# yanglei18/SGV3D

Measured on AMD Instinct MI355X. Metric: camera frames/sec at 864x1536->BEV, higher is better.
Workload: dtype f32

## Files before the change

### include/sgv3d_hip.h

```cpp
#ifndef SGV3D_HIP_H
#define SGV3D_HIP_H

#include <stddef.h>
#include <stdint.h>

#ifdef __cplusplus
extern "C" {
#endif

#define SGV3D_OK 0
#define SGV3D_EINVAL (-1)
#define SGV3D_ELAUNCH (-2)
#define SGV3D_ENOSPACE (-3)

const char *sgv3d_last_error(void);
int sgv3d_abi_version(void);


int sgv3d_voxel_pooling_forward(int batch_size, int num_points, int num_channels,
                                int num_voxel_x, int num_voxel_y, int num_voxel_z,
                                const int32_t *geom_xyz, const float *input_features,
                                float *output_features, int32_t *pos_memo, void *stream);
int sgv3d_voxel_pooling_forward_fresh(int batch_size, int num_points, int num_channels,
                                      int num_voxel_x, int num_voxel_y, int num_voxel_z,
// ... 112 lines not shown

#define SGV3D_TILE_128x128 1
#define SGV3D_TILE_128x64 2
#define SGV3D_TILE_64x128 3
#define SGV3D_TILE_64x64 4
#define SGV3D_TILE_32x128 9
#define SGV3D_TILE_48x64 10
#define SGV3D_TILE_X3 64
#define SGV3D_TILE_MFIRST 16
#define SGV3D_TILE_OCC5 32
#define SGV3D_WINOGRAD_RESIDENT 6
#define SGV3D_WINOGRAD_HALF 8

int sgv3d_conv_winograd4_pack_weight(const float *w_src , int cout, int cin, int k_pad, int cout_pad,
                                     float *u_packed , void *stream);
int sgv3d_conv_winograd4_pack_weight_x3(const float *w_src, int cout, int cin, int cin_pad, int cout_pad, void *u3_packed,
                                        void *stream);

int sgv3d_conv_pack_weight_x3(const float *w_src, int cout, int cin, int kh, int kw, int cin_pad, int cout_pad, void *u3_packed,
                              void *stream);
int sgv3d_conv2d_x3_forward(const sgv3d_conv_desc *desc, const float *x, const void *u3_packed, const float *scale,
                            const float *bias, const float *residual, float *y, void *workspace, size_t workspace_bytes,
                            void *stream);
int sgv3d_conv2d_x3_shortcut_forward(const sgv3d_conv_desc *desc_a, const float *xa, const void *u3a, const float *scale_a,
                                     const float *bias_a, const sgv3d_conv_desc *desc_b, const float *xb, const void *u3b,
                                     const float *scale_b, const float *bias_b, float *y, void *stream);
int sgv3d_stem_pool_x3_forward(int batch, int h, int w, const float *x_nchw, const void *w_x3, size_t w_bytes, const float *scale,
                               const float *shift, float *y_nhwc, int y_ld, int variant, void *stream);
int sgv3d_wino4_lattice_axis(int n, int dil, int tile, int k0, int count, int *tiles, int *stacked, int *pixels);
size_t sgv3d_conv2d_winograd4_workspace_bytes(const sgv3d_conv_desc *desc );
int sgv3d_conv2d_winograd4_forward(const sgv3d_conv_desc *desc , const float *x, const float *u_packed,
                                   const float *scale, const float *bias, const float *residual, float *y,
                                   void *workspace, size_t workspace_bytes, void *stream);

size_t sgv3d_conv2d_winograd4_multi_workspace_bytes(int n, const sgv3d_conv_desc *descs );
int sgv3d_conv2d_winograd4_forward_multi(int n, const sgv3d_conv_desc *descs , const float *x, const void *const *u_packed,
                                         const float *const *scale, const float *const *bias, float *const *y, void *workspace,
                                         size_t workspace_bytes, void *stream);

void sgv3d_conv_pack_geometry(int k, int n, int *k_pad, int *n_pad);

int sgv3d_conv_pack_weight(const float *w_src, int cout, int cin, int kh, int kw, int cin_pad,
                           int transposed, int k_order, float *w_packed, int k_pad, int cout_pad,
                           void *stream);

size_t sgv3d_conv2d_workspace_bytes(const sgv3d_conv_desc *desc );
// ... 660 lines not shown
```

### sgv3d_amd/_lib.py

```python
import ctypes
import os

_HERE = os.path.dirname(os.path.abspath(__file__))
LIB_PATH = os.path.join(_HERE, "csrc", "libsgv3d_hip.so")

c_int, c_void_p, c_size_t, c_ll = ctypes.c_int, ctypes.c_void_p, ctypes.c_size_t, ctypes.c_longlong


class ConvDesc(ctypes.Structure):
    _fields_ = [(n, c_int) for n in (
        "batch", "in_h", "in_w", "cin", "out_h", "out_w", "cout", "kh", "kw", "stride", "pad", "dil",
        "x_ld", "x_coff", "y_ld", "y_coff", "res_ld", "relu", "mode", "deconv_ks", "k_pad", "cout_pad",
        "tile", "x_nchw", "k_order", "split_k")]


class VitAttnDesc(ctypes.Structure):
    _fields_ = [(n, c_int) for n in ("batch", "height", "width", "heads", "head_dim", "win_h", "win_w")]


class SamAttnDesc(ctypes.Structure):
    _fields_ = [(n, c_int) for n in ("batch", "nq", "nk", "heads", "head_dim", "q_ld", "k_ld", "v_ld", "o_ld")] + [("scale", ctypes.c_float)]


CONV_NORMAL, CONV_DECONV, CONV_NCHW_OUT, CONV_GROUP_PLANES = 0, 1, 2, 3
# ... 59 lines not shown
    "sgv3d_scale_channels_bf16": (c_int, [c_int] * 3 + [c_void_p] * 4),
    "sgv3d_global_avgpool_bf16": (c_int, [c_int] * 4 + [c_void_p] * 3 + [c_size_t, c_void_p]),
    "sgv3d_broadcast_channels_bf16": (c_int, [c_int] * 5 + [c_void_p] * 3),
    "sgv3d_upsample_bilinear2x_bf16": (c_int, [c_int] * 4 + [c_void_p] * 3),
    "sgv3d_add_mul_sigmoid_bf16": (c_int, [c_ll] + [c_void_p] * 5),
    "sgv3d_deform_im2col3x3_bf16": (c_int, [c_int] * 5 + [c_void_p] * 2 + [c_int, c_void_p, c_void_p]),
    "sgv3d_conv3x3_patch_bf16_weight_bytes": (c_size_t, [c_int, c_int]),
    "sgv3d_conv3x3_patch_bf16_debug_stamps": (None, [c_void_p]),
    "sgv3d_conv3x3_patch_bf16_pack_weight": (c_int, [c_void_p, c_int, c_int, c_void_p, c_void_p]),
    "sgv3d_conv3x3_patch_bf16_forward": (c_int, [c_int] * 11 + [c_void_p] * 6 + [c_int, c_int, c_void_p, c_size_t, c_void_p]),
    "sgv3d_conv_dw_bf16_weight_bytes": (c_size_t, [c_int] * 4),
    "sgv3d_conv_dw_bf16_pack_weight": (c_int, [c_void_p] + [c_int] * 5 + [c_void_p, c_void_p]),
    "sgv3d_conv_dw_bf16_forward": (c_int, [ctypes.POINTER(ConvDesc)] + [c_void_p] * 7),
    "sgv3d_conv_dw_bf16_workspace_bytes": (c_size_t, [ctypes.POINTER(ConvDesc)]),
    "sgv3d_conv_dw_bf16_forward_splitk": (c_int, [ctypes.POINTER(ConvDesc)] + [c_void_p] * 7 + [c_size_t, c_void_p]),
    "sgv3d_conv_dw_bf16_pair_forward": (c_int, [ctypes.POINTER(ConvDesc)] + [c_void_p] * 4 + [c_int] + [c_void_p] * 4 + [c_int, c_void_p, c_int, c_int, c_int, c_void_p]),
    "sgv3d_conv_winograd_weight_floats": (c_size_t, [c_int, c_int]),
    "sgv3d_conv_winograd_pack_weight": (c_int, [c_void_p, c_int, c_int, c_int, c_void_p, c_void_p]),
    "sgv3d_conv2d_winograd_forward": (c_int, [ctypes.POINTER(ConvDesc)] + [c_void_p] * 8 + [c_size_t, c_void_p]),
    "sgv3d_conv_winograd4_pack_weight": (c_int, [c_void_p, c_int, c_int, c_int, c_int, c_void_p, c_void_p]),
    "sgv3d_conv_winograd4_pack_weight_x3": (c_int, [c_void_p, c_int, c_int, c_int, c_int, c_void_p, c_void_p]),
    "sgv3d_conv_pack_weight_x3": (c_int, [c_void_p, c_int, c_int, c_int, c_int, c_int, c_int, c_void_p, c_void_p]),
    "sgv3d_conv2d_x3_forward": (c_int, [c_void_p] * 8 + [c_size_t, c_void_p]),
    "sgv3d_conv2d_x3_shortcut_forward": (c_int, [c_void_p] * 12),
    "sgv3d_stem_pool_x3_forward": (c_int, [c_int] * 3 + [c_void_p, c_void_p, c_size_t] + [c_void_p] * 3 + [c_int, c_int, c_void_p]),
    "sgv3d_wino4_lattice_axis": (c_int, [c_int] * 5 + [c_void_p] * 3),
    "sgv3d_conv2d_winograd4_workspace_bytes": (c_size_t, [ctypes.POINTER(ConvDesc)]),
    "sgv3d_conv2d_winograd4_forward": (c_int, [ctypes.POINTER(ConvDesc)] + [c_void_p] * 7 + [c_size_t, c_void_p]),
    "sgv3d_conv2d_winograd4_multi_workspace_bytes": (c_size_t, [c_int, c_void_p]),
    "sgv3d_conv2d_winograd4_forward_multi": (c_int, [c_int] + [c_void_p] * 7 + [c_size_t, c_void_p]),
    "sgv3d_maxpool3x3s2": (c_int, [c_int] * 4 + [c_void_p] * 3),
    "sgv3d_maxpool3x3s2_bf16": (c_int, [c_int] * 4 + [c_void_p] * 3),
    "sgv3d_nchw_to_nhwc": (c_int, [c_int] * 5 + [c_void_p] * 3),
    "sgv3d_nhwc_to_nchw": (c_int, [c_int] * 6 + [c_void_p] * 3),
    "sgv3d_global_avgpool_workspace_bytes": (c_size_t, [c_int] * 2),
    "sgv3d_global_avgpool": (c_int, [c_int] * 4 + [c_void_p] * 3 + [c_size_t, c_void_p]),
    "sgv3d_dense": (c_int, [c_int] * 3 + [c_void_p] * 4 + [c_int, c_void_p, c_void_p]),
    "sgv3d_broadcast_channels": (c_int, [c_int] * 5 + [c_void_p] * 3),
    "sgv3d_scale_channels": (c_int, [c_int] * 3 + [c_void_p] * 4),
    "sgv3d_copy_channels": (c_int, [c_int] * 5 + [c_void_p] * 3),
    "sgv3d_upsample_bilinear2x": (c_int, [c_int] * 4 + [c_void_p] * 3),
    "sgv3d_add_mul_sigmoid": (c_int, [c_ll] + [c_void_p] * 5),
    "sgv3d_bsm_compose": (c_int, [c_int] * 6 + [c_void_p, c_int, ctypes.c_float, c_void_p, c_void_p]),
    "sgv3d_deform_im2col3x3": (c_int, [c_int] * 5 + [c_void_p, c_void_p, c_int, c_void_p, c_void_p]),
    "sgv3d_deform_conv3x3_forward": (c_int, [c_int] * 6 + [c_void_p, c_void_p, c_int, c_void_p, c_int, c_int, c_void_p, c_int, c_int,
                                                          c_void_p]),
# ... 226 lines not shown
```

### sgv3d_amd/csrc/conv_pw_x3.hip

```cpp
#include "conv_common.hpp"
#include "f32x3.hpp"

using namespace sgv3d;

namespace {

struct PwX3Args {
    const float *x, *scale, *bias, *res;
    const void *w;
    float *y;
    int M, K, N;
    int x_ld, x_coff, y_ld, y_coff, res_ld, relu;
    int cout_pad, tiles_m, tiles_n, mfirst;
    unsigned x_bytes, w_bytes;
    int in_h, in_w, out_h, out_w, kh, kw, stride, pad, dil;
    int cin4;
    int split_k;
    float *ws;
    const float *x2, *scale2, *bias2;
    const void *w2;
    int K2, x2_ld, x2_coff;
    unsigned x2_bytes, w2_bytes;
};

template <int MA, int WN, int MODE>
__global__ __launch_bounds__(64 * WN, 2) void conv_pw_x3_kernel(const PwX3Args a) {
    constexpr bool TAPS = MODE == 1, TM = MODE == 2, DUAL = MODE == 3, DECONV = MODE == 4;
    constexpr int NT = 64 * WN, BM = 16 * MA, BN = 32 * WN;
    constexpr int PLANE = x3_plane_bytes(BM), BUF = x3_buf_bytes(BM);
    __shared__ __attribute__((aligned(16))) unsigned char smem[2 * BUF];

    const int logical = xcd_tile(blockIdx.x, a.tiles_m * a.tiles_n);
    int tn, tm;
    if (a.mfirst) {
        tm = (int)((unsigned)logical / (unsigned)a.tiles_n);
        tn = logical - tm * a.tiles_n;
    } else {
        tn = (int)((unsigned)logical / (unsigned)a.tiles_m);
        tm = logical - tn * a.tiles_m;
    }
    const int m0 = tm * BM, n0 = tn * BN;
    const int kb = a.K >> 5;

    const int tid = threadIdx.x;
    __amdgpu_buffer_rsrc_t x_rsrc = __builtin_amdgcn_make_buffer_rsrc(const_cast<float *>(a.x), 0, (int)a.x_bytes, 0x00020000);
    __amdgpu_buffer_rsrc_t w_rsrc = __builtin_amdgcn_make_buffer_rsrc(const_cast<void *>(a.w), 0, (int)a.w_bytes, 0x00020000);
// ... 150 lines not shown
#pragma unroll
        for (int i = 0; i < PA; ++i) {
            const int r = arow + RPA * i;
            const bool live = a_on[i] && m0 + r < a.M;
            const int m = live ? m0 + r : 0;
            const int t = (int)((unsigned)m / (unsigned)a.out_w);
            const int ow = m - t * a.out_w;
            const int n = (int)((unsigned)t / (unsigned)a.out_h);
            const int oh = t - n * a.out_h;
            xg[i] = live ? (unsigned)((((long long)(n * a.in_h + oh * a.stride) * a.in_w + ow * a.stride) * a.x2_ld + a.x2_coff + ach * 4) * 4)
                         : 0xffffffffu;
        }
#pragma unroll
        for (int nb = 0; nb < 2; ++nb) wgo[nb] = u3_lane_offset((n0 >> 4) + 2 * wave + nb, nkt, lane, a.cout_pad);
        __syncthreads();
        PWX3_KLOOP();
    }
#undef PWX3_KLOOP
#undef PWX3_REQUEST
#undef PWX3_STORE

    if (a.split_k > 1) {
        float *wsb = a.ws + (size_t)blockIdx.y * a.M * a.N;
#pragma unroll
        for (int nb = 0; nb < 2; ++nb) {
            const int col = n0 + 32 * wave + 16 * nb + 4 * g;
            if (col >= a.N) continue;
#pragma unroll
            for (int ma = 0; ma < MA; ++ma) {
                const int row = m0 + 16 * ma + l16;
                if (row < a.M) *reinterpret_cast<f32x4 *>(wsb + (size_t)row * a.N + col) = acc[ma][nb];
            }
        }
        return;
    }
    const float floor_ = a.relu ? 0.f : -__builtin_inff();
    if constexpr (DUAL) {
#pragma unroll
        for (int nb = 0; nb < 2; ++nb) {
            const int col = n0 + 32 * wave + 16 * nb + 4 * g;
            if (col >= a.N) continue;
            const f32x4 sc = a.scale2 ? *reinterpret_cast<const f32x4 *>(a.scale2 + col) : f32x4{1.f, 1.f, 1.f, 1.f};
            const f32x4 sh = a.bias2 ? *reinterpret_cast<const f32x4 *>(a.bias2 + col) : f32x4{0.f, 0.f, 0.f, 0.f};
#pragma unroll
            for (int ma = 0; ma < MA; ++ma) {
                const int row = m0 + 16 * ma + l16;
                if (row >= a.M) continue;
                const f32x4 u = acc[ma][nb] * sc + sh;
                f32x4 v = tkeep[ma][nb];
                v += u;
                v = f32x4{fmaxf(v[0], floor_), fmaxf(v[1], floor_), fmaxf(v[2], floor_), fmaxf(v[3], floor_)};
                *reinterpret_cast<f32x4 *>(a.y + (size_t)row * a.y_ld + a.y_coff + col) = v;
            }
        }
// ... 67 lines not shown
    if (mode == 4) hipLaunchKernelGGL((conv_pw_x3_kernel<MA, WN, 4>), grid, dim3(64 * WN), 0, st, a);
    else if (mode == 3) hipLaunchKernelGGL((conv_pw_x3_kernel<MA, WN, 3>), grid, dim3(64 * WN), 0, st, a);
    else if (mode == 2) hipLaunchKernelGGL((conv_pw_x3_kernel<MA, WN, 2>), grid, dim3(64 * WN), 0, st, a);
    else if (mode == 1) hipLaunchKernelGGL((conv_pw_x3_kernel<MA, WN, 1>), grid, dim3(64 * WN), 0, st, a);
    else hipLaunchKernelGGL((conv_pw_x3_kernel<MA, WN, 0>), grid, dim3(64 * WN), 0, st, a);
    return check_launch("conv_pw_x3_kernel");
}

}

extern "C" int sgv3d_conv_pack_weight_x3(const float *w_src, int cout, int cin, int kh, int kw, int cin_pad, int cout_pad, void *u3_packed,
                                         void *stream) {
    const int k_order = cin_pad % 32 == 0 ? 1 : 0;
    SGV3D_REQUIRE(w_src && u3_packed && cout > 0 && cin > 0 && kh > 0 && kw > 0 && kh * kw <= (k_order ? 32 : 64) && cin_pad >= cin &&
                      cin_pad % 4 == 0 && cout_pad >= cout && cout_pad % 32 == 0,
                  "conv_pack_weight_x3: bad arguments (cout=%d cin=%d k=%dx%d cin_pad=%d cout_pad=%d)", cout, cin, kh, kw, cin_pad, cout_pad);
    const long long kp = k_order ? (long long)cin_pad * kh * kw : ((long long)cin_pad * kh * kw + 31) / 32 * 32;
    const long long total = (long long)cout_pad * kp;
    hipLaunchKernelGGL(pack_weight_x3_kernel, dim3(cdiv(total, 256)), dim3(256), 0, as_stream(stream), w_src, cout, cin, cin_pad, cout_pad,
                       kh * kw, k_order, static_cast<__bf16 *>(u3_packed));
    return check_launch("pack_weight_x3_kernel");
}

extern "C" int sgv3d_conv2d_x3_forward(const sgv3d_conv_desc *d, const float *x, const void *u3_packed, const float *scale,
                                       const float *bias, const float *residual, float *y, void *workspace, size_t workspace_bytes,
                                       void *stream) {
    SGV3D_REQUIRE(d && x && u3_packed && y, "conv2d_x3_forward: null pointer");
    const bool tapmajor = d->cin % 32 != 0;
    const bool deconv = d->mode == SGV3D_CONV_DECONV;
    if (deconv) {
        SGV3D_REQUIRE(d->kh == 1 && d->kw == 1 && d->stride == 1 && d->pad == 0 && d->deconv_ks >= 1 && d->deconv_ks <= 64 &&
                          residual == nullptr,
                      "conv2d_x3_forward: DECONV runs as a 1x1 GEMM with deconv_ks = kernel = stride (<= 64), no residual");
        SGV3D_REQUIRE(d->in_h > 0 && d->in_w > 0 && d->out_h == d->in_h * d->deconv_ks && d->out_w == d->in_w * d->deconv_ks,
                      "conv2d_x3_forward: DECONV output must be input * deconv_ks");
        SGV3D_REQUIRE(d->cin > 0 && d->cin % 32 == 0 && d->cout > 0 && d->cout % 4 == 0 &&
                          (long long)d->cout * d->deconv_ks * d->deconv_ks <= 0x1000000LL,
                      "conv2d_x3_forward: DECONV needs cin %% 32 == 0, cout %% 4 == 0 (cin=%d cout=%d)", d->cin, d->cout);
        SGV3D_REQUIRE((long long)d->batch * d->out_h * d->out_w < 0x7fffffffLL, "conv2d_x3_forward: DECONV output has 2^31 pixels or more");
    }
    SGV3D_REQUIRE((deconv || d->mode == SGV3D_CONV_NORMAL) && d->kh > 0 && d->kw > 0 && d->kh * d->kw <= (tapmajor ? 64 : 32) && d->stride > 0 &&
                      d->dil > 0 && d->pad >= 0,
                  "conv2d_x3_forward: NHWC output, at most 32 taps (64 with tap-major weights)");
    SGV3D_REQUIRE(d->batch > 0 && d->in_h > 0 && d->in_w > 0 && d->cin > 0 && d->cout > 0 && d->cin % 4 == 0 && d->cout % 4 == 0,
                  "conv2d_x3_forward: cin %% 4 == 0, cout %% 4 == 0 (cin=%d cout=%d)", d->cin, d->cout);
    SGV3D_REQUIRE(deconv || (d->out_h == (d->in_h + 2 * d->pad - d->dil * (d->kh - 1) - 1) / d->stride + 1 &&
                                 d->out_w == (d->in_w + 2 * d->pad - d->dil * (d->kw - 1) - 1) / d->stride + 1),
                  "conv2d_x3_forward: output size does not match the geometry");
    SGV3D_REQUIRE((d->x_ld & 3) == 0 && (d->x_coff & 3) == 0 && (d->y_ld & 3) == 0 && (d->y_coff & 3) == 0 && (residual == nullptr || (d->res_ld & 3) == 0),
// ... 4 lines not shown
    SGV3D_REQUIRE(d->cout_pad >= gemm_n && d->cout_pad % 32 == 0, "conv2d_x3_forward: desc.cout_pad = rows of the x3 weights (a multiple of 32)");
    SGV3D_REQUIRE(((reinterpret_cast<uintptr_t>(x) | reinterpret_cast<uintptr_t>(y) | reinterpret_cast<uintptr_t>(residual) |
                    reinterpret_cast<uintptr_t>(scale) | reinterpret_cast<uintptr_t>(bias) | reinterpret_cast<uintptr_t>(u3_packed)) & 15) == 0,
                  "conv2d_x3_forward: pointers must be 16-B aligned");
    const long long M = deconv ? (long long)d->batch * d->in_h * d->in_w : (long long)d->batch * d->out_h * d->out_w;
    const long long K = tapmajor ? ((long long)d->kh * d->kw * d->cin + 31) / 32 * 32 : (long long)d->kh * d->kw * d->cin;
    const long long xb = (long long)d->batch * d->in_h * d->in_w * d->x_ld * 4, wb = (long long)d->cout_pad * K * 6;
    SGV3D_REQUIRE(M < 0x7fffffffLL && xb < 0xf0000000LL && wb < 0xf0000000LL, "conv2d_x3_forward: operands larger than 3.75 GiB");
    const int variant = d->tile & 15;
    SGV3D_REQUIRE((d->tile & SGV3D_TILE_X3) && (variant & 3) < 3 && (variant & 12) != 12,
                  "conv2d_x3_forward: desc.tile = SGV3D_TILE_X3 | variant, variant in {0,1,2, 4,5,6, 8,9,10}");
    const int taps = deconv ? 4 : tapmajor ? 2 : (d->kh == 1 && d->kw == 1 && d->stride == 1 && d->pad == 0) ? 0 : 1;
    PwX3Args a;
    a.x = x; a.w = u3_packed; a.scale = scale; a.bias = bias; a.res = residual; a.y = y;
    a.M = (int)M; a.K = (int)K; a.N = gemm_n;
    a.x_ld = d->x_ld; a.x_coff = d->x_coff; a.y_ld = d->y_ld; a.y_coff = d->y_coff; a.res_ld = d->res_ld; a.relu = d->relu;
    a.cout_pad = d->cout_pad;
    a.mfirst = (d->tile & SGV3D_TILE_MFIRST) ? 1 : 0;
    a.x_bytes = (unsigned)xb; a.w_bytes = (unsigned)wb;
    a.in_h = d->in_h; a.in_w = d->in_w; a.out_h = d->out_h; a.out_w = d->out_w;
    a.kh = d->kh; a.kw = d->kw; a.stride = d->stride; a.pad = d->pad; a.dil = d->dil;
    a.cin4 = d->cin / 4;
    if (deconv) { a.kh = d->deconv_ks; a.cin4 = d->cout; }
    const int bm = 32 << (variant & 3), bn = (variant & 8) ? 256 : (variant & 4) ? 64 : 128;
    a.tiles_m = (int)cdiv(M, bm);
    a.tiles_n = cdiv(gemm_n, bn);
    hipStream_t st = as_stream(stream);
    a.split_k = d->split_k > 1 ? d->split_k : 1;
    a.ws = nullptr;
    if (a.split_k > 1) {
        SGV3D_REQUIRE(a.split_k <= K / 32, "conv2d_x3_forward: split_k %d exceeds the %lld k-steps", a.split_k, K / 32);
        const size_t need = (size_t)a.split_k * (size_t)M * gemm_n * sizeof(float);
        if (!workspace || workspace_bytes < need)
            return fail(SGV3D_ENOSPACE, "conv2d_x3_forward: split-K workspace has %zu bytes, needs %zu", workspace_bytes, need);
        SGV3D_REQUIRE((reinterpret_cast<uintptr_t>(workspace) & 15) == 0, "conv2d_x3_forward: workspace must be 16-B aligned");
        a.ws = static_cast<float *>(workspace);
    }
    int rc;
    switch (variant) {
        case 0: rc = launch_pw<2, 4>(a, taps, st); break;
        case 1: rc = launch_pw<4, 4>(a, taps, st); break;
        case 2: rc = launch_pw<8, 4>(a, taps, st); break;
        case 4: rc = launch_pw<2, 2>(a, taps, st); break;
        case 5: rc = launch_pw<4, 2>(a, taps, st); break;
        case 6: rc = launch_pw<8, 2>(a, taps, st); break;
        case 8: rc = launch_pw<2, 8>(a, taps, st); break;
        case 9: rc = launch_pw<4, 8>(a, taps, st); break;
        default: rc = launch_pw<8, 8>(a, taps, st); break;
    }
    if (rc != SGV3D_OK || a.split_k <= 1) return rc;
    ConvArgs r{};
    r.M = a.M; r.N = a.N; r.ws = a.ws; r.split_k = a.split_k;
    r.scale = scale; r.bias = bias; r.res = residual; r.res_ld = d->res_ld; r.relu = d->relu;
    r.y = y; r.y_ld = d->y_ld; r.y_coff = d->y_coff; r.mode = d->mode; r.ks = d->deconv_ks; r.cout = d->cout;
    r.m_h = deconv ? d->in_h : d->out_h; r.m_w = deconv ? d->in_w : d->out_w; r.out_h = d->out_h; r.out_w = d->out_w;
    return launch_splitk_reduce(r, st);
}

extern "C" int sgv3d_conv2d_x3_shortcut_forward(const sgv3d_conv_desc *da, const float *xa, const void *u3a, const float *scale_a,
                                                const float *bias_a, const sgv3d_conv_desc *db, const float *xb, const void *u3b,
                                                const float *scale_b, const float *bias_b, float *y, void *stream) {
    SGV3D_REQUIRE(da && db && xa && xb && u3a && u3b && y, "conv2d_x3_shortcut_forward: null pointer");
    SGV3D_REQUIRE(da->mode == SGV3D_CONV_NORMAL && db->mode == SGV3D_CONV_NORMAL && da->split_k <= 1 && db->split_k <= 1,
                  "conv2d_x3_shortcut_forward: NHWC output, no split-K");
    SGV3D_REQUIRE(da->kh == 1 && da->kw == 1 && da->stride == 1 && da->pad == 0 && db->kh == 1 && db->kw == 1 && db->pad == 0 &&
                      (db->stride == 1 || db->stride == 2),
                  "conv2d_x3_shortcut_forward: source A is 1x1 / stride 1, source B 1x1 / stride 1 or 2, neither padded");
    SGV3D_REQUIRE(da->batch > 0 && da->in_h > 0 && da->in_w > 0 && db->in_h > 0 && db->in_w > 0 && da->cin > 0 && db->cin > 0 &&
                      da->cout > 0 && da->cin % 32 == 0 && db->cin % 32 == 0 && da->cout % 4 == 0,
                  "conv2d_x3_shortcut_forward: cin %% 32 == 0 on both sources, cout %% 4 == 0 (cin=%d / %d cout=%d)", da->cin, db->cin,
                  da->cout);
    SGV3D_REQUIRE(da->cout == db->cout && da->cout_pad == db->cout_pad, "conv2d_x3_shortcut_forward: the sources' cout differ (%d / %d)",
                  da->cout, db->cout);
    SGV3D_REQUIRE(da->out_h == da->in_h && da->out_w == da->in_w && db->out_h == (db->in_h - 1) / db->stride + 1 &&
                      db->out_w == (db->in_w - 1) / db->stride + 1,
                  "conv2d_x3_shortcut_forward: output size does not match the geometry");
    SGV3D_REQUIRE(da->batch == db->batch && da->out_h == db->out_h && da->out_w == db->out_w,
                  "conv2d_x3_shortcut_forward: the sources' output geometries differ (%dx%dx%d / %dx%dx%d)", da->batch, da->out_h,
                  da->out_w, db->batch, db->out_h, db->out_w);
// ... 51 lines not shown
```

### sgv3d_amd/hip_ops.py

```python
import ctypes
from collections import namedtuple
from functools import partialmethod

import torch

from . import _lib, conv_tiles, pack_cache
from ._lib import ConvDesc, CONV_NORMAL, CONV_DECONV, CONV_NCHW_OUT, CONV_GROUP_PLANES
from .conv_tiles import (TILE_WINO, TILE_WINO_RES, TILE_PATCH, TILE_WINO_HALF, TILE_WINO4, TILE_WINO4_WIDE, TILE_WINO4_NARROW,
                         TILE_WINO4_OCC, TILE_WINO4_G48, TILE_F4RES)


def _st(t):
    return _lib.stream_handle(t.device)


PROFILE = None
AUTOTUNE = not __import__("os").environ.get("SGV3D_NO_AUTOTUNE")
DETERMINISTIC = __import__("os").environ.get("SGV3D_DETERMINISTIC", "0") not in ("", "0")


def deterministic():
    return DETERMINISTIC or torch.are_deterministic_algorithms_enabled()
PROFILE_DETAIL = False
import os as _os
TUNE_STREAMS = max(1, int(_os.environ.get("SGV3D_TUNE_STREAMS", "1")))
TUNE_VERBOSE = bool(_os.environ.get("SGV3D_TUNE_VERBOSE"))
TUNE_ROUNDS = max(1, int(_os.environ.get("SGV3D_TUNE_ROUNDS", "3")))
TUNE_REPEATS = max(1, int(_os.environ.get("SGV3D_TUNE_REPEATS", "2")))
SPLIT_K = not _os.environ.get("SGV3D_NO_SPLITK")
# ... 673 lines not shown
                                                 out.data_ptr(), _lib.ptr(ws), nws, _st(x))

    def _launch_winograd4(self, lib, T, d, x, tail, gate, out, io, ws, nws):
        if not self.wino4_ok(d, gate) or d.split_k > 1:
            raise _lib.SGV3DError("F(4x4) Winograd covers f32 3x3 / stride 1 / pad 1 layers with cin % 32 == 0, cout % 4 == 0, "
                                  "NHWC output, no gate, no split-K")
        u = self._form(T.form)
        a = self._abi(d, T, self.cin, self.wino4_x3_cout_pad) if T.x3 else self._abi(d, T, *self.wino4_geom)
        nws4 = lib.sgv3d_conv2d_winograd4_workspace_bytes(a)
        ws4 = torch.empty(nws4, dtype=torch.uint8, device=x.device)
        return lib.sgv3d_conv2d_winograd4_forward(a, x.data_ptr(), u.data_ptr(), *tail, out.data_ptr(), ws4.data_ptr(), nws4, _st(x))

    def _launch_f4res(self, lib, T, d, x, tail, gate, out, io, ws, nws):
        if not self.f4res_ok(d, gate, io) or d.split_k > 1 or x.dtype != torch.float32:
            raise _lib.SGV3DError("the resident F(4x4) kernel covers f32 3x3 / stride 1 / pad 1 layers with 64 input channels "
                                  "(cout % 64 == 0) or 64 output channels (cin % 64 == 0), NHWC output, no gate, no split-K")
        return lib.sgv3d_conv3x3_f4res_forward(self._abi(d, T), x.data_ptr(), self._form(T.form).data_ptr(), *tail, out.data_ptr(), _st(x))

    def _launch_x3(self, lib, T, d, x, tail, gate, out, io, ws, nws):
        if not self.pw_x3_ok(d, gate, io) or x.dtype != torch.float32:
            raise _lib.SGV3DError("the implicit-GEMM f32x3 kernel covers f32 layers with at most 32 taps, cin % 32 == 0 (>= 64), cout % 4 == 0, "
                                  "NHWC output, no gate")
        u = self._form(T.form)
        return lib.sgv3d_conv2d_x3_forward(self._abi(d, T, d.k_pad, self.pw_x3_cout_pad), x.data_ptr(), u.data_ptr(), *tail, out.data_ptr(),
                                           _lib.ptr(ws), nws, _st(x))

    def _launch_patch_bf16(self, lib, T, d, x, tail, gate, out, io, ws, nws):
        if not self._patch_eligible(d, gate):
            raise _lib.SGV3DError("the bf16 patch kernel covers 3x3 / stride 1 / pad 1 layers with cin % 32 == 0 in bf16 mode")
        return lib.sgv3d_conv3x3_patch_bf16_forward(d.batch, d.in_h, d.in_w, self.cin, self.cout, d.x_ld, d.x_coff, d.y_ld,
                                                    d.y_coff, d.res_ld, d.relu, x.data_ptr(), self._patch_weights().data_ptr(),
                                                    *tail, out.data_ptr(), int(io), int(d.split_k), _lib.ptr(ws), nws, _st(x))

    def _launch_dw_bf16(self, lib, T, d, x, tail, gate, out, io, ws, nws):
        if not self._dw_eligible(d, gate, io) or (d.split_k > 1 and d.mode != CONV_NORMAL):
            raise _lib.SGV3DError("the bf16 direct-weight kernel covers layers with cin % 32 == 0, cout % 8 == 0 and bf16 tensors in "
                                  "and out (NHWC), no gate; split-K in NORMAL mode only")
        if d.split_k > 1:
            nws = lib.sgv3d_conv_dw_bf16_workspace_bytes(ctypes.byref(d))
            ws = torch.empty(nws, dtype=torch.uint8, device=x.device)
            return lib.sgv3d_conv_dw_bf16_forward_splitk(self._abi(d, T), x.data_ptr(), self._dw_weights().data_ptr(), *tail,
                                                         out.data_ptr(), ws.data_ptr(), nws, _st(x))
        return lib.sgv3d_conv_dw_bf16_forward(self._abi(d, T), x.data_ptr(), self._dw_weights().data_ptr(), *tail, out.data_ptr(), _st(x))

    def _time_under_load(self, lib, d, x, residual, gate, out, rounds=None, io=0):
        global _TUNE_SIDE_STREAMS
        cur = torch.cuda.current_stream(x.device)
        if len(_TUNE_SIDE_STREAMS) < TUNE_STREAMS:
# ... 103 lines not shown
        with torch.cuda.device(x.device):
            for t, splits in cands:
                for sk in splits:
                    d.tile, d.split_k = t, sk
                    _lib.check(self._launch(lib, d, x, residual, gate, out, io), "sgv3d_conv2d_forward")
                    if TUNE_STREAMS > 1:
                        dt = self._time_under_load(lib, d, x, residual, gate, out, io=io)
                    else:
                        nrep = max(4, TUNE_ROUNDS * TUNE_REPEATS // 2)
                        evs = [torch.cuda.Event(enable_timing=True) for _ in range(nrep + 1)]
                        evs[0].record()
                        for r in range(nrep):
                            self._launch(lib, d, x, residual, gate, out, io)
                            evs[r + 1].record()
                        evs[-1].synchronize()
                        dt = min(evs[r].elapsed_time(evs[r + 1]) for r in range(nrep))
                    if TUNE_VERBOSE:
                        print(f"[tune] {self.cout}x{self.cin}k{self.kh} {d.batch}x{d.in_h}x{d.in_w}: tile {t} split {sk}: {dt * 1e3:.1f} us", flush=True)
                    if best_t is None or dt < best_t:
                        best, best_t = (t, sk), dt
        return best


PAIR_BF16 = _os.environ.get("SGV3D_PAIR_BF16", "1") != "0"


PARALLEL_BRANCHES = _os.environ.get("SGV3D_PARALLEL_BRANCHES", "0") == "1"
_BRANCH_POOL = {}
_BRANCH_TOP = {}


_OWNED_STREAMS = {}


def distinct_stream(device, avoid=()):
    dev = torch.device(device)
    key = dev.index if dev.index is not None else torch.cuda.current_device()
    taken = _OWNED_STREAMS.setdefault(key, set())
    banned = {st.cuda_stream for st in avoid if st is not None} | {torch.cuda.current_stream(dev).cuda_stream} | taken
    for _ in range(64):
        st = torch.cuda.Stream(device=dev)
        if st.cuda_stream not in banned:
            if len(taken) < 24:
                taken.add(st.cuda_stream)
            return st
    return torch.cuda.Stream(device=dev)
# ... 326 lines not shown
        raise _lib.SGV3DError(f"deconv_x3: tile {T.id} is not a tile of the f32x3 pointwise kernel")
    u = conv._form("w_pw_x3_deconv")
    d = ConvDesc()
    d.batch, d.in_h, d.in_w, d.cin = B, H, W, conv.cin
    d.out_h, d.out_w, d.cout = oh, ow, conv.cout
    d.kh, d.kw, d.stride, d.pad, d.dil = 1, 1, 1, 0, 1
    d.x_ld, d.x_coff, d.y_ld, d.y_coff, d.res_ld = x_ld, 0, int(out.shape[-1]), int(y_coff), 0
    d.relu, d.mode, d.deconv_ks, d.split_k, d.tile = (1 if conv.relu else 0), CONV_DECONV, conv.ks, sk, T.abi
    d.k_pad, d.cout_pad, d.k_order = conv.cin, conv.pw_x3_deconv_cout_pad, 1
    ws, nws = None, 0
    if sk > 1:
        nws = 4 * sk * gemm_m * gemm_n
        ws = torch.empty(nws, dtype=torch.uint8, device=x.device)
    real_n = conv.cout_real * conv.ks * conv.ks
    flops = 2.0 * gemm_m * real_n * conv.cin_real
    nbytes = 4.0 * (gemm_m * conv.cin_real + real_n * conv.cin_real + gemm_m * real_n)
    name, extra = "conv_pw_x3_deconv", None
    if PROFILE_DETAIL:
        name += f"|{B}x{H}x{W}x{conv.cin}->{conv.cout} k{-conv.ks} s1 d1 splitk{sk}"
    if PROFILE is not None:
        mfma = 2.0 * gemm_m * gemm_n * conv.cin
        extra = {"symbol": f"conv_pw_x3_kernel<{T.bm // 16}, {T.bn // 32}, 4>", "mfma_flops": mfma, "bf16_mfma_flops": 6 * mfma}
    with torch.cuda.device(x.device), prof(name, flops, nbytes, extra):
        rc = _lib.load().sgv3d_conv2d_x3_forward(ctypes.byref(d), x.data_ptr(), u.data_ptr(), _lib.ptr(conv.scale), _lib.ptr(conv.shift),
                                                 None, out.data_ptr(), _lib.ptr(ws), nws, _st(x))
    _lib.check(rc, "sgv3d_conv2d_x3_forward")
    return out


def deconv_x3_signature(conv, x):
    B, H, W, _ = (int(v) for v in x.shape)
    return f"pair|deconv|{conv.cout}x{conv.cin}ks{conv.ks}|{B}x{H}x{W}|r{int(conv.relu)}|ts{TUNE_STREAMS}"


def deconv_x3_choice(conv, x, out=None, y_coff=0):
    if not deconv_x3_eligible(conv, x, out, y_coff):
        return None
    B, H, W, _ = (int(v) for v in x.shape)
    gemm_m, gemm_n, nkt = B * H * W, conv.ks * conv.ks * conv.cout, conv.cin // 32
    rule = _deconv_x3_rule(gemm_m, gemm_n)
    sig = deconv_x3_signature(conv, x)
    hit = tune_lookup(sig, x.device)
    if hit is not None:
        on, code = (int(v) for v in hit)
        if not on:
            return None
        sk, t = divmod(code, 100)
        ok = t in PW_X3_TILES and not TILES[t].mfirst and 1 <= sk <= max(1, nkt) and (sk == 1 or SPLIT_K)
# ... 510 lines not shown
```

### sgv3d_amd/pipeline.py

```python
import os
import warnings

import torch

from . import hip_ops
from .calibration import CalibrationCache, tensor_version

from ._lib import SGV3DError
CAPTURE_ERRORS = (RuntimeError, SGV3DError)
FORK_REFRESH = os.environ.get("SGV3D_GRAPH_FORK_REFRESH", "0") == "1"


class eager_forward:

    def __init__(self, model):
        self.model = model

    def __enter__(self):
        self.saved = getattr(self.model, "_graph_suspended", 0)
        self.model._graph_suspended = self.saved + 1
        return self

    def __exit__(self, *exc):
        self.model._graph_suspended = self.saved
        return False


def static_copy(t):
# ... 23 lines not shown
        return type(obj)(_clone_aliased(v, memo) for v in obj)
    return obj


class GraphedForward:

    def __init__(self, model, imgs, mats):
        dev = imgs.device
        self.in_imgs = static_copy(imgs)
        self.in_mats = {k: static_copy(v) for k, v in mats.items()}
        self._mat_keys = sorted(self.in_mats)
        self._mat_dst = [self.in_mats[k] for k in self._mat_keys]
        self.cache = CalibrationCache()
        self.replays = 0
        self.decoded = None
        side = hip_ops.distinct_stream(dev)
        branch = hip_ops.distinct_stream(dev, (side,))
        self._streams = (side, branch)
        cur = torch.cuda.current_stream(dev)
        side.wait_stream(cur)
        own = model.backbone.calib_cache
        model.backbone.calib_cache = self.cache
        sweeps = range(int(self.in_imgs.shape[1]))
        try:
            with torch.cuda.stream(side), torch.no_grad(), eager_forward(model):
                preds = model(self.in_imgs, self.in_mats)
                model.head.decode_device(preds)
                del preds
                side.synchronize()
                self.graphs = [torch.cuda.CUDAGraph()]
                pool = torch.cuda.graph_pool_handle()
                split = os.environ.get("SGV3D_GRAPH_SPLIT", "1") != "0"

                def fork_refresh():
                    if not FORK_REFRESH:
                        self.cache.invalidate()
                        for sweep in sweeps:
                            model.backbone.calibration(self.in_mats, sweep)
                        return
                    branch.wait_stream(side)
                    with torch.cuda.stream(branch):
                        self.cache.invalidate()
                        for sweep in sweeps:
                            model.backbone.calibration(self.in_mats, sweep)
                    for sweep in sweeps:
                        self.cache.entry(sweep).join_stream = branch

                def cut(tag):
# ... 56 lines not shown
        for _ in range(self.slots):
            self.streams.append(hip_ops.distinct_stream(self.device, self.streams))
        if decode is not None:
            from .jpeg import JpegStaging
            self.stagings = [JpegStaging(decode, tuple(mats['sensor2ego_mats'].shape[:3])) for _ in range(self.slots)]
            with torch.no_grad():
                for st in self.stagings:
                    st.stage(imgs)
                    st.launch()
            self.in_frames = [st.out for st in self.stagings]
            with torch.no_grad():
                self.in_imgs = [preprocess(f)[0] for f in self.in_frames]
            imgs = self.in_imgs[0]
        elif preprocess is None:
            self.in_frames = None
            self.in_imgs = [static_copy(imgs) for _ in range(self.slots)]
        else:
            self.in_frames = [static_copy(imgs) for _ in range(self.slots)]
            with torch.no_grad():
                self.in_imgs = [preprocess(f)[0] for f in self.in_frames]
            imgs = self.in_imgs[0]
        self.in_mats = [{k: static_copy(v) for k, v in mats.items()} for _ in range(self.slots)]
        self.caches = [CalibrationCache() for _ in range(self.slots)]
        self._last_mats = [None] * self.slots
        self.outputs = [None] * self.slots
        self.graphs = []
        self.done = [torch.cuda.Event() for _ in range(self.slots)]
        self._next = 0
        self._own_cache = model.backbone.calib_cache
        with torch.no_grad(), eager_forward(model):
            model(imgs, mats)
            torch.cuda.synchronize(imgs.device)
            if use_graph:
                try:
                    for i, s in enumerate(self.streams):
                        g = torch.cuda.CUDAGraph()
                        s.wait_stream(torch.cuda.current_stream(imgs.device))
                        with torch.cuda.stream(s), self._slot(i):
                            self._forward(i)
                            torch.cuda.synchronize(imgs.device)
                            with torch.inference_mode(False), torch.no_grad(), torch.cuda.graph(g, stream=s):
                                self.outputs[i] = self._forward(i)
                        torch.cuda.current_stream(imgs.device).wait_stream(s)
                        self.graphs.append(g)
                except CAPTURE_ERRORS as e:
                    self.graphs = []
                    self.outputs = [None] * self.slots
                    self.capture_error = e
                    torch.cuda.synchronize(imgs.device)
                    if strict:
                        raise
                    warnings.warn(f"FramePipeline: hipGraph capture failed ({type(e).__name__}: {e}); running eager launches on "
                                  f"the slot streams instead (pass strict=True to raise)", RuntimeWarning, stacklevel=2)
        self.use_graph = bool(self.graphs)

    def __del__(self):
        for st in getattr(self, 'streams', ()):
            hip_ops.release_stream(st)

    class _Slot:
        def __init__(self, pipe, i):
            self.pipe, self.i = pipe, i

        def __enter__(self):
            self.pipe.model.backbone.calib_cache = self.pipe.caches[self.i]

        def __exit__(self, *exc):
            self.pipe.model.backbone.calib_cache = self.pipe._own_cache
            return False

    def _forward(self, i):
        if self.stagings is not None:
            self.stagings[i].launch()
        if self.preprocess is not None:
            self.preprocess(self.in_frames[i], out=self.in_imgs[i])
        return self.model(self.in_imgs[i], self.in_mats[i])

    def _slot(self, i):
        return FramePipeline._Slot(self, i)

    def replay(self, slot=None):
        i = self._next if slot is None else slot
        self._next = (i + 1) % self.slots
        with torch.cuda.stream(self.streams[i]), torch.no_grad():
            if self.graphs:
                self.graphs[i].replay()
            else:
                with self._slot(i), eager_forward(self.model):
                    self.outputs[i] = self._forward(i)
            self.done[i].record()
# ... 38 lines not shown
```

Before: 299.7.

## Fuse split-K reduction into the f32x3 pointwise conv via arrival counters

Split-K partials for the f32x3 implicit-GEMM conv are now reduced inside the same launch: each tile's last-arriving k-slice block, found through an atomic per-tile counter, sums the slabs and applies the epilogue. This removes the separate split-K reduce kernel launch and its extra pass over the workspace for layers with small slabs. Per-slot and per-stream counter arenas are added so graph capture and multiple streams stay safe. The cost is an atomic and a barrier in every block, plus a serial combine tail done by one block per tile.

```diff
diff --git a/include/sgv3d_hip.h b/include/sgv3d_hip.h
--- a/include/sgv3d_hip.h
+++ b/include/sgv3d_hip.h
@@ -158,6 +158,10 @@
 int sgv3d_conv2d_x3_forward(const sgv3d_conv_desc *desc, const float *x, const void *u3_packed, const float *scale,
                             const float *bias, const float *residual, float *y, void *workspace, size_t workspace_bytes,
                             void *stream);
+size_t sgv3d_conv2d_x3_counters_bytes(const sgv3d_conv_desc *desc);
+int sgv3d_conv2d_x3_forward_counters(const sgv3d_conv_desc *desc, const float *x, const void *u3_packed, const float *scale,
+                                     const float *bias, const float *residual, float *y, void *workspace, size_t workspace_bytes,
+                                     void *counters, size_t counters_bytes, void *stream);
 int sgv3d_conv2d_x3_shortcut_forward(const sgv3d_conv_desc *desc_a, const float *xa, const void *u3a, const float *scale_a,
                                      const float *bias_a, const sgv3d_conv_desc *desc_b, const float *xb, const void *u3b,
                                      const float *scale_b, const float *bias_b, float *y, void *stream);
diff --git a/sgv3d_amd/_lib.py b/sgv3d_amd/_lib.py
--- a/sgv3d_amd/_lib.py
+++ b/sgv3d_amd/_lib.py
@@ -105,6 +105,8 @@
     "sgv3d_conv_winograd4_pack_weight_x3": (c_int, [c_void_p, c_int, c_int, c_int, c_int, c_void_p, c_void_p]),
     "sgv3d_conv_pack_weight_x3": (c_int, [c_void_p, c_int, c_int, c_int, c_int, c_int, c_int, c_void_p, c_void_p]),
     "sgv3d_conv2d_x3_forward": (c_int, [c_void_p] * 8 + [c_size_t, c_void_p]),
+    "sgv3d_conv2d_x3_counters_bytes": (c_size_t, [ctypes.POINTER(ConvDesc)]),
+    "sgv3d_conv2d_x3_forward_counters": (c_int, [c_void_p] * 8 + [c_size_t, c_void_p, c_size_t, c_void_p]),
     "sgv3d_conv2d_x3_shortcut_forward": (c_int, [c_void_p] * 12),
     "sgv3d_stem_pool_x3_forward": (c_int, [c_int] * 3 + [c_void_p, c_void_p, c_size_t] + [c_void_p] * 3 + [c_int, c_int, c_void_p]),
     "sgv3d_wino4_lattice_axis": (c_int, [c_int] * 5 + [c_void_p] * 3),
diff --git a/sgv3d_amd/csrc/conv_pw_x3.hip b/sgv3d_amd/csrc/conv_pw_x3.hip
--- a/sgv3d_amd/csrc/conv_pw_x3.hip
+++ b/sgv3d_amd/csrc/conv_pw_x3.hip
@@ -1,5 +1,6 @@
 #include "conv_common.hpp"
 #include "f32x3.hpp"
+#include "splitk_combine.hpp"
 
 using namespace sgv3d;
 
@@ -17,11 +18,57 @@
     int cin4;
     int split_k;
     float *ws;
+    unsigned *cnt;
     const float *x2, *scale2, *bias2;
     const void *w2;
     int K2, x2_ld, x2_coff;
     unsigned x2_bytes, w2_bytes;
 };
+
+
+template <int MA, int S, bool DECONV>
+__device__ __forceinline__ void pw_x3_combine(const PwX3Args &a, int m0, int col0, int l16) {
+    constexpr int RB0 = S <= 2 ? 4 : S <= 5 ? 2 : 1, RB = RB0 < MA ? RB0 : MA;
+    static_assert(MA % RB == 0, "whole batches of m-rows");
+    const unsigned slab = (unsigned)(a.M * a.N) * 4u;
+    __amdgpu_buffer_rsrc_t ws = __builtin_amdgcn_make_buffer_rsrc(a.ws, 0, (int)(S * slab), 0x00020000);
+    [[maybe_unused]] ConvArgs e{};
+    if constexpr (DECONV) {
+        e.M = a.M; e.N = a.N; e.scale = a.scale; e.bias = a.bias; e.relu = a.relu;
+        e.y = a.y; e.y_ld = a.y_ld; e.y_coff = a.y_coff; e.mode = SGV3D_CONV_DECONV; e.ks = a.kh; e.cout = a.cin4;
+        e.m_h = a.in_h; e.m_w = a.in_w; e.out_h = a.out_h; e.out_w = a.out_w;
+    }
+#pragma unroll 1
+    for (int ma0 = 0; ma0 < MA; ma0 += RB) {
+        sk_f32x4 t[RB][2][S];
+#pragma unroll
+        for (int r = 0; r < RB; ++r) {
+            const int row = m0 + 16 * (ma0 + r) + l16;
+#pragma unroll
+            for (int nb = 0; nb < 2; ++nb) {
+                const int col = col0 + 16 * nb;
+                const bool on = row < a.M && col < a.N;
+                splitk_load4<S>(ws, on ? (unsigned)(row * a.N + col) * 4u : 0u, slab, t[r][nb]);
+            }
+        }
+#pragma unroll
+        for (int r = 0; r < RB; ++r) {
+            const int row = m0 + 16 * (ma0 + r) + l16;
+#pragma unroll
+            for (int nb = 0; nb < 2; ++nb) {
+                const int col = col0 + 16 * nb;
+                if (row >= a.M || col >= a.N) continue;
+                const sk_f32x4 v = splitk_sum4<S>(t[r][nb]);
+                if constexpr (DECONV) {
+#pragma unroll 1
+                    for (int j = 0; j < 4; ++j) conv_epilogue_store(e, row, col + j, j == 0 ? v.x : j == 1 ? v.y : j == 2 ? v.z : v.w);
+                } else {
+                    splitk_store4(v, a.scale, a.bias, a.res, a.res_ld, a.relu, a.y, a.y_ld, a.y_coff, (unsigned)row, (unsigned)col);
+                }
+            }
+        }
+    }
+}
 
 template <int MA, int WN, int MODE>
 __global__ __launch_bounds__(64 * WN, 2) void conv_pw_x3_kernel(const PwX3Args a) {
@@ -218,14 +265,42 @@
 
     if (a.split_k > 1) {
         float *wsb = a.ws + (size_t)blockIdx.y * a.M * a.N;
-#pragma unroll
-        for (int nb = 0; nb < 2; ++nb) {
-            const int col = n0 + 32 * wave + 16 * nb + 4 * g;
-            if (col >= a.N) continue;
-#pragma unroll
-            for (int ma = 0; ma < MA; ++ma) {
-                const int row = m0 + 16 * ma + l16;
-                if (row < a.M) *reinterpret_cast<f32x4 *>(wsb + (size_t)row * a.N + col) = acc[ma][nb];
+        const bool one_launch = !DUAL && a.cnt != nullptr;
+        if (one_launch) {
+            __amdgpu_buffer_rsrc_t slab = __builtin_amdgcn_make_buffer_rsrc(wsb, 0, a.M * a.N * 4, 0x00020000);
+#pragma unroll
+            for (int nb = 0; nb < 2; ++nb) {
+                const int col = n0 + 32 * wave + 16 * nb + 4 * g;
+                if (col >= a.N) continue;
+#pragma unroll
+                for (int ma = 0; ma < MA; ++ma) {
+                    const int row = m0 + 16 * ma + l16;
+                    if (row < a.M) splitk_store_partial4(slab, (unsigned)(row * a.N + col) * 4u, acc[ma][nb]);
+                }
+            }
+        } else {
+#pragma unroll
+            for (int nb = 0; nb < 2; ++nb) {
+                const int col = n0 + 32 * wave + 16 * nb + 4 * g;
+                if (col >= a.N) continue;
+#pragma unroll
+                for (int ma = 0; ma < MA; ++ma) {
+                    const int row = m0 + 16 * ma + l16;
+                    if (row < a.M) *reinterpret_cast<f32x4 *>(wsb + (size_t)row * a.N + col) = acc[ma][nb];
+                }
+            }
+        }
+        if constexpr (!DUAL) {
+            if (!one_launch || !splitk_arrive(a.cnt + blockIdx.x, a.split_k, smem, (wave | l16 | g) == 0)) return;
+            const int col0 = n0 + 32 * wave + 4 * g;
+            switch (a.split_k) {
+                case 2: pw_x3_combine<MA, 2, DECONV>(a, m0, col0, l16); break;
+                case 3: pw_x3_combine<MA, 3, DECONV>(a, m0, col0, l16); break;
+                case 4: pw_x3_combine<MA, 4, DECONV>(a, m0, col0, l16); break;
+                case 5: pw_x3_combine<MA, 5, DECONV>(a, m0, col0, l16); break;
+                case 6: pw_x3_combine<MA, 6, DECONV>(a, m0, col0, l16); break;
+                case 7: pw_x3_combine<MA, 7, DECONV>(a, m0, col0, l16); break;
+                default: pw_x3_combine<MA, 8, DECONV>(a, m0, col0, l16); break;
             }
         }
         return;
@@ -339,9 +414,16 @@
     return check_launch("pack_weight_x3_kernel");
 }
 
-extern "C" int sgv3d_conv2d_x3_forward(const sgv3d_conv_desc *d, const float *x, const void *u3_packed, const float *scale,
-                                       const float *bias, const float *residual, float *y, void *workspace, size_t workspace_bytes,
-                                       void *stream) {
+namespace {
+
+inline void pw_x3_tile_shape(int variant, int &bm, int &bn) {
+    bm = 32 << (variant & 3);
+    bn = (variant & 8) ? 256 : (variant & 4) ? 64 : 128;
+}
+
+int conv2d_x3_forward_impl(const sgv3d_conv_desc *d, const float *x, const void *u3_packed, const float *scale, const float *bias,
+                           const float *residual, float *y, void *workspace, size_t workspace_bytes, void *counters,
+                           size_t counters_bytes, void *stream) {
     SGV3D_REQUIRE(d && x && u3_packed && y, "conv2d_x3_forward: null pointer");
     const bool tapmajor = d->cin % 32 != 0;
     const bool deconv = d->mode == SGV3D_CONV_DECONV;
@@ -392,12 +474,23 @@
     a.kh = d->kh; a.kw = d->kw; a.stride = d->stride; a.pad = d->pad; a.dil = d->dil;
     a.cin4 = d->cin / 4;
     if (deconv) { a.kh = d->deconv_ks; a.cin4 = d->cout; }
-    const int bm = 32 << (variant & 3), bn = (variant & 8) ? 256 : (variant & 4) ? 64 : 128;
+    int bm, bn;
+    pw_x3_tile_shape(variant, bm, bn);
     a.tiles_m = (int)cdiv(M, bm);
     a.tiles_n = cdiv(gemm_n, bn);
     hipStream_t st = as_stream(stream);
     a.split_k = d->split_k > 1 ? d->split_k : 1;
     a.ws = nullptr;
+    a.cnt = nullptr;
+    if (a.split_k > 1 && counters) {
+        SGV3D_REQUIRE(a.split_k <= kSplitKOneLaunchMax && a.split_k * M * gemm_n < 0x20000000LL,
+                      "conv2d_x3_forward_counters: the one-launch form covers split_k <= %d (got %d)", kSplitKOneLaunchMax, a.split_k);
+        const size_t need = (size_t)a.tiles_m * a.tiles_n * sizeof(unsigned);
+        if (counters_bytes < need)
+            return fail(SGV3D_ENOSPACE, "conv2d_x3_forward_counters: %zu bytes of counters, needs %zu", counters_bytes, need);
+        SGV3D_REQUIRE((reinterpret_cast<uintptr_t>(counters) & 3) == 0, "conv2d_x3_forward_counters: counters must be 4-B aligned");
+        a.cnt = static_cast<unsigned *>(counters);
+    }
     if (a.split_k > 1) {
         SGV3D_REQUIRE(a.split_k <= K / 32, "conv2d_x3_forward: split_k %d exceeds the %lld k-steps", a.split_k, K / 32);
         const size_t need = (size_t)a.split_k * (size_t)M * gemm_n * sizeof(float);
@@ -418,13 +511,44 @@
         case 9: rc = launch_pw<4, 8>(a, taps, st); break;
         default: rc = launch_pw<8, 8>(a, taps, st); break;
     }
-    if (rc != SGV3D_OK || a.split_k <= 1) return rc;
+    if (rc != SGV3D_OK || a.split_k <= 1 || a.cnt) return rc;
     ConvArgs r{};
     r.M = a.M; r.N = a.N; r.ws = a.ws; r.split_k = a.split_k;
     r.scale = scale; r.bias = bias; r.res = residual; r.res_ld = d->res_ld; r.relu = d->relu;
     r.y = y; r.y_ld = d->y_ld; r.y_coff = d->y_coff; r.mode = d->mode; r.ks = d->deconv_ks; r.cout = d->cout;
     r.m_h = deconv ? d->in_h : d->out_h; r.m_w = deconv ? d->in_w : d->out_w; r.out_h = d->out_h; r.out_w = d->out_w;
     return launch_splitk_reduce(r, st);
+}
+
+}
+
+extern "C" int sgv3d_conv2d_x3_forward(const sgv3d_conv_desc *d, const float *x, const void *u3_packed, const float *scale,
+                                       const float *bias, const float *residual, float *y, void *workspace, size_t workspace_bytes,
+                                       void *stream) {
+    return conv2d_x3_forward_impl(d, x, u3_packed, scale, bias, residual, y, workspace, workspace_bytes, nullptr, 0, stream);
+}
+
+extern "C" size_t sgv3d_conv2d_x3_counters_bytes(const sgv3d_conv_desc *d) {
+    if (!d || d->split_k <= 1 || d->split_k > kSplitKOneLaunchMax || d->batch <= 0 || d->in_h <= 0 || d->in_w <= 0 || d->out_h <= 0 ||
+        d->out_w <= 0 || d->cout <= 0)
+        return 0;
+    const bool deconv = d->mode == SGV3D_CONV_DECONV;
+    if (!deconv && d->mode != SGV3D_CONV_NORMAL) return 0;
+    if (deconv && d->deconv_ks < 1) return 0;
+    const int variant = d->tile & 15;
+    if (!(d->tile & SGV3D_TILE_X3) || (variant & 3) == 3 || (variant & 12) == 12) return 0;
+    const long long M = deconv ? (long long)d->batch * d->in_h * d->in_w : (long long)d->batch * d->out_h * d->out_w;
+    const long long N = deconv ? (long long)d->cout * d->deconv_ks * d->deconv_ks : d->cout;
+    if (M >= 0x7fffffffLL || N > 0x1000000LL || d->split_k * M * N >= 0x20000000LL) return 0;
+    int bm, bn;
+    pw_x3_tile_shape(variant, bm, bn);
+    return (size_t)(cdiv(M, bm) * cdiv(N, (long long)bn)) * sizeof(unsigned);
+}
+
+extern "C" int sgv3d_conv2d_x3_forward_counters(const sgv3d_conv_desc *d, const float *x, const void *u3_packed, const float *scale,
+                                                const float *bias, const float *residual, float *y, void *workspace,
+                                                size_t workspace_bytes, void *counters, size_t counters_bytes, void *stream) {
+    return conv2d_x3_forward_impl(d, x, u3_packed, scale, bias, residual, y, workspace, workspace_bytes, counters, counters_bytes, stream);
 }
 
 extern "C" int sgv3d_conv2d_x3_shortcut_forward(const sgv3d_conv_desc *da, const float *xa, const void *u3a, const float *scale_a,
diff --git a/sgv3d_amd/csrc/splitk_combine.hpp b/sgv3d_amd/csrc/splitk_combine.hpp
--- /dev/null
+++ b/sgv3d_amd/csrc/splitk_combine.hpp
@@ -0,0 +1,59 @@
+#pragma once
+#include "conv_common.hpp"
+
+namespace sgv3d {
+
+typedef float sk_f32x4 __attribute__((ext_vector_type(4)));
+
+constexpr int kSplitKOneLaunchMax = 8;
+
+static __device__ __forceinline__ bool splitk_arrive(unsigned *counter, int split_k, void *lds_word, bool leader) {
+    volatile unsigned *flag = static_cast<volatile unsigned *>(lds_word);
+    asm volatile("s_waitcnt vmcnt(0)" ::: "memory");
+    __syncthreads();
+    if (leader) {
+        const unsigned ticket = __hip_atomic_fetch_add(counter, 1u, __ATOMIC_RELAXED, __HIP_MEMORY_SCOPE_AGENT);
+        const bool last = ticket == (unsigned)split_k - 1u;
+        if (last) {
+            __hip_atomic_store(counter, 0u, __ATOMIC_RELAXED, __HIP_MEMORY_SCOPE_AGENT);
+        }
+        *flag = last ? 1u : 0u;
+    }
+    __syncthreads();
+    return *flag != 0u;
+}
+
+typedef unsigned sk_u32x4 __attribute__((ext_vector_type(4)));
+static __device__ __forceinline__ void splitk_store_partial4(__amdgpu_buffer_rsrc_t slab, unsigned byte_offset, sk_f32x4 v) {
+    __builtin_amdgcn_raw_buffer_store_b128(__builtin_bit_cast(sk_u32x4, v), slab, (int)byte_offset, 0, 16);
+}
+
+template <int S>
+static __device__ __forceinline__ void splitk_load4(__amdgpu_buffer_rsrc_t ws, unsigned byte_offset, unsigned slab_bytes, sk_f32x4 (&t)[S]) {
+#pragma unroll
+    for (int s = 0; s < S; ++s)
+        t[s] = __builtin_bit_cast(sk_f32x4, __builtin_amdgcn_raw_buffer_load_b128(ws, (int)byte_offset, (int)(s * slab_bytes), 16));
+}
+
+template <int S>
+static __device__ __forceinline__ sk_f32x4 splitk_sum4(const sk_f32x4 (&t)[S]) {
+    sk_f32x4 v = {0.f, 0.f, 0.f, 0.f};
+#pragma unroll
+    for (int s = 0; s < S; ++s) { v.x += t[s].x; v.y += t[s].y; v.z += t[s].z; v.w += t[s].w; }
+    return v;
+}
+
+static __device__ __forceinline__ void splitk_store4(sk_f32x4 v, const float *scale, const float *bias, const float *res, int res_ld,
+                                                     int relu, float *y, int y_ld, int y_coff, unsigned row, unsigned col) {
+    const sk_f32x4 sc = scale ? *reinterpret_cast<const sk_f32x4 *>(scale + col) : sk_f32x4{1.f, 1.f, 1.f, 1.f};
+    const sk_f32x4 sh = bias ? *reinterpret_cast<const sk_f32x4 *>(bias + col) : sk_f32x4{0.f, 0.f, 0.f, 0.f};
+    v.x = v.x * sc.x + sh.x; v.y = v.y * sc.y + sh.y; v.z = v.z * sc.z + sh.z; v.w = v.w * sc.w + sh.w;
+    if (res) {
+        const sk_f32x4 r = *reinterpret_cast<const sk_f32x4 *>(res + (size_t)row * res_ld + col);
+        v.x += r.x; v.y += r.y; v.z += r.z; v.w += r.w;
+    }
+    if (relu) { v.x = fmaxf(v.x, 0.f); v.y = fmaxf(v.y, 0.f); v.z = fmaxf(v.z, 0.f); v.w = fmaxf(v.w, 0.f); }
+    *reinterpret_cast<sk_f32x4 *>(y + (size_t)row * y_ld + y_coff + col) = v;
+}
+
+}
diff --git a/sgv3d_amd/hip_ops.py b/sgv3d_amd/hip_ops.py
--- a/sgv3d_amd/hip_ops.py
+++ b/sgv3d_amd/hip_ops.py
@@ -4,7 +4,7 @@
 
 import torch
 
-from . import _lib, conv_tiles, pack_cache
+from . import _lib, conv_tiles, pack_cache, splitk_counters
 from ._lib import ConvDesc, CONV_NORMAL, CONV_DECONV, CONV_NCHW_OUT, CONV_GROUP_PLANES
 from .conv_tiles import (TILE_WINO, TILE_WINO_RES, TILE_PATCH, TILE_WINO_HALF, TILE_WINO4, TILE_WINO4_WIDE, TILE_WINO4_NARROW,
                          TILE_WINO4_OCC, TILE_WINO4_G48, TILE_F4RES)
@@ -724,8 +724,7 @@
             raise _lib.SGV3DError("the implicit-GEMM f32x3 kernel covers f32 layers with at most 32 taps, cin % 32 == 0 (>= 64), cout % 4 == 0, "
                                   "NHWC output, no gate")
         u = self._form(T.form)
-        return lib.sgv3d_conv2d_x3_forward(self._abi(d, T, d.k_pad, self.pw_x3_cout_pad), x.data_ptr(), u.data_ptr(), *tail, out.data_ptr(),
-                                           _lib.ptr(ws), nws, _st(x))
+        return _x3_forward(lib, self._abi(d, T, d.k_pad, self.pw_x3_cout_pad), x, u, tail, out, ws, nws)
 
     def _launch_patch_bf16(self, lib, T, d, x, tail, gate, out, io, ws, nws):
         if not self._patch_eligible(d, gate):
@@ -875,6 +874,24 @@
         return best
 
 
+def _x3_forward(lib, a, x, u, tail, out, ws, nws):
+    if a._obj.split_k > 1:
+        arena, need = None, 0
+        if x.is_cuda and splitk_counters.ONE_LAUNCH:
+            d = a._obj
+            v = d.tile & 15
+            gemm_n = d.cout * d.deconv_ks * d.deconv_ks if d.mode == CONV_DECONV else d.cout
+            small = splitk_counters.slab_bytes(d.split_k, 32 << (v & 3), 256 if v & 8 else 64 if v & 4 else 128, gemm_n) <= splitk_counters.MAX_SLAB_BYTES
+            need = int(lib.sgv3d_conv2d_x3_counters_bytes(a)) if small else 0
+            if need:
+                arena = splitk_counters.lookup(x.device, _st(x), torch.cuda.is_current_stream_capturing(), need)
+        splitk_counters.STATS["one_launch" if arena is not None else "two_launch"] += 1
+        if arena is not None:
+            return lib.sgv3d_conv2d_x3_forward_counters(a, x.data_ptr(), u.data_ptr(), *tail, out.data_ptr(), _lib.ptr(ws), nws,
+                                                        arena.ptr(), need, _st(x))
+    return lib.sgv3d_conv2d_x3_forward(a, x.data_ptr(), u.data_ptr(), *tail, out.data_ptr(), _lib.ptr(ws), nws, _st(x))
+
+
 PAIR_BF16 = _os.environ.get("SGV3D_PAIR_BF16", "1") != "0"
 
 
@@ -1247,8 +1264,7 @@
         mfma = 2.0 * gemm_m * gemm_n * conv.cin
         extra = {"symbol": f"conv_pw_x3_kernel<{T.bm // 16}, {T.bn // 32}, 4>", "mfma_flops": mfma, "bf16_mfma_flops": 6 * mfma}
     with torch.cuda.device(x.device), prof(name, flops, nbytes, extra):
-        rc = _lib.load().sgv3d_conv2d_x3_forward(ctypes.byref(d), x.data_ptr(), u.data_ptr(), _lib.ptr(conv.scale), _lib.ptr(conv.shift),
-                                                 None, out.data_ptr(), _lib.ptr(ws), nws, _st(x))
+        rc = _x3_forward(_lib.load(), ctypes.byref(d), x, u, (_lib.ptr(conv.scale), _lib.ptr(conv.shift), None), out, ws, nws)
     _lib.check(rc, "sgv3d_conv2d_x3_forward")
     return out
 
diff --git a/sgv3d_amd/pipeline.py b/sgv3d_amd/pipeline.py
--- a/sgv3d_amd/pipeline.py
+++ b/sgv3d_amd/pipeline.py
@@ -3,7 +3,7 @@
 
 import torch
 
-from . import hip_ops
+from . import hip_ops, splitk_counters
 from .calibration import CalibrationCache, tensor_version
 
 from ._lib import SGV3DError
@@ -73,8 +73,10 @@
         own = model.backbone.calib_cache
         model.backbone.calib_cache = self.cache
         sweeps = range(int(self.in_imgs.shape[1]))
+        with torch.cuda.stream(side):
+            self.splitk_arena = splitk_counters.new_arena(dev)
         try:
-            with torch.cuda.stream(side), torch.no_grad(), eager_forward(model):
+            with torch.cuda.stream(side), torch.no_grad(), eager_forward(model), splitk_counters.bind(self.splitk_arena, side.cuda_stream):
                 preds = model(self.in_imgs, self.in_mats)
                 model.head.decode_device(preds)
                 del preds
@@ -177,6 +179,7 @@
             imgs = self.in_imgs[0]
         self.in_mats = [{k: static_copy(v) for k, v in mats.items()} for _ in range(self.slots)]
         self.caches = [CalibrationCache() for _ in range(self.slots)]
+        self.splitk_arenas = [splitk_counters.new_arena(self.device) for _ in range(self.slots)]
         self._last_mats = [None] * self.slots
         self.outputs = [None] * self.slots
         self.graphs = []
@@ -219,8 +222,11 @@
 
         def __enter__(self):
             self.pipe.model.backbone.calib_cache = self.pipe.caches[self.i]
+            self.bound = splitk_counters.bind(self.pipe.splitk_arenas[self.i], self.pipe.streams[self.i].cuda_stream)
+            self.bound.__enter__()
 
         def __exit__(self, *exc):
+            self.bound.__exit__(*exc)
             self.pipe.model.backbone.calib_cache = self.pipe._own_cache
             return False
 
diff --git a/sgv3d_amd/splitk_counters.py b/sgv3d_amd/splitk_counters.py
--- /dev/null
+++ b/sgv3d_amd/splitk_counters.py
@@ -0,0 +1,83 @@
+import os
+import threading
+
+ONE_LAUNCH = os.environ.get("SGV3D_SPLITK_ONE_LAUNCH", "1") != "0"
+ARENA_BYTES = 4 * 4096
+MAX_SLAB_BYTES = int(os.environ.get("SGV3D_SPLITK_ONE_LAUNCH_MAX_SLAB", str(64 << 10)))
+STATS = {"one_launch": 0, "two_launch": 0}
+
+_EAGER = {}
+_LOCK = threading.Lock()
+_BOUND = threading.local()
+
+
+def _zeros(nbytes, device):
+    import torch
+    return torch.zeros(nbytes, dtype=torch.uint8, device=device)
+
+
+def _index(device):
+    idx = getattr(device, "index", None)
+    return device if idx is None else int(idx)
+
+
+class Arena:
+
+    def __init__(self, device, nbytes=ARENA_BYTES, alloc=None):
+        self.device = device
+        self.nbytes = int(nbytes)
+        self.buf = (alloc or _zeros)(self.nbytes, device)
+
+    def ptr(self):
+        return self.buf.data_ptr()
+
+
+class bind:
+
+    def __init__(self, arena, stream_handle):
+        self.item = None if arena is None else (arena, int(stream_handle))
+
+    def __enter__(self):
+        if self.item is not None:
+            if not hasattr(_BOUND, "stack"):
+                _BOUND.stack = []
+            _BOUND.stack.append(self.item)
+        return self
+
+    def __exit__(self, *exc):
+        if self.item is not None:
+            top = _BOUND.stack.pop()
+            assert top is self.item, "splitk_counters.bind contexts must nest"
+        return False
+
+
+def slab_bytes(split_k, bm, bn, gemm_n):
+    return int(split_k) * int(bm) * min(int(bn), int(gemm_n)) * 4
+
+
+def new_arena(device, alloc=None):
+    return Arena(device, ARENA_BYTES, alloc) if ONE_LAUNCH else None
+
+
+def lookup(device, stream_handle, capturing, need_bytes, alloc=None):
+    if not ONE_LAUNCH or need_bytes <= 0:
+        return None
+    stream_handle = int(stream_handle)
+    stack = getattr(_BOUND, "stack", None)
+    if stack:
+        arena, bound_stream = stack[-1]
+        if bound_stream == stream_handle and _index(arena.device) == _index(device):
+            return arena if need_bytes <= arena.nbytes else None
+    if capturing:
+        return None
+    key = (_index(device), stream_handle)
+    with _LOCK:
+        arena = _EAGER.get(key)
+        if arena is None:
+            arena = _EAGER[key] = Arena(device, ARENA_BYTES, alloc)
+    return arena if need_bytes <= arena.nbytes else None
+
+
+def reset():
+    with _LOCK:
+        _EAGER.clear()
```

Result: no change. 299.5 (median of 2 runs) (-0.1%).
